# myshell-ai/OpenVoice

Measured on NVIDIA H100. Metric: audio_seconds_per_second, higher is better.
Workload: dtype f32 (3xFP16 split-precision tensor-core convs with fp32 accumulation, fp32 FFMA elsewhere)

## Files before the change

### include/ovc.h

```cpp
#ifndef OVC_B200_H
#define OVC_B200_H

#include <stddef.h>
#include <stdint.h>

#ifdef __cplusplus
extern "C" {
#endif

#define OVC_ABI_VERSION 17

#if defined(__GNUC__)
#define OVC_API __attribute__((visibility("default")))
#else
#define OVC_API
#endif

enum {
  OVC_OK = 0,
  OVC_ERR_INVALID = -1,
  OVC_ERR_CUDA = -2,
  OVC_ERR_STATE = -3,
  OVC_ERR_MISSING = -4,
  OVC_ERR_NOMEM = -5
};
// ... 154 lines not shown
                                      float* d_stats, int32_t* d_cum, float* d_g, int64_t* d_y_lengths, void* stream);
OVC_API int ovc_tts_decode_windows_tokens(ovc_ctx* ctx, const float* stats, const int32_t* cum, const float* g,
                                          const int64_t* y_lengths, int N, int T, const int64_t* row, const int64_t* frame0,
                                          const int64_t* len, int W, int Wmax, const uint64_t* seed, const int64_t* stream,
                                          const float* noise_scale, float* o, float* z_p, void* cuda_stream);

OVC_API int ovc_set_precision(ovc_ctx* ctx, int mode);

#define OVC_OPT_TTS_SIMPLE 2
#define OVC_OPT_GRAPH 3
#define OVC_OPT_PDL 5
#define OVC_OPT_BRANCHES 7
#define OVC_OPT_PAIR 8
#define OVC_OPT_PAIR_OCC 9
#define OVC_OPT_STAGED_EPI 10
OVC_API int ovc_set_option(ovc_ctx* ctx, int key, int value);

OVC_API int ovc_last_launch_count(const ovc_ctx* ctx);

OVC_API int ovc_graph_replays(const ovc_ctx* ctx);

OVC_API int ovc_profile_enable(ovc_ctx* ctx, int enable);
OVC_API int ovc_profile_read(ovc_ctx* ctx, double* ms, int64_t* launches, double* flops, double* bytes);
OVC_API int ovc_profile_detail(ovc_ctx* ctx, int max, char* names, double* ms, double* flops, double* bytes,
                               int* family);

OVC_API int ovc_debug_enable(ovc_ctx* ctx, int enable);
OVC_API int ovc_debug_fetch(ovc_ctx* ctx, const char* name, float* host_out, size_t max_floats,
                    int64_t* shape4 );

// ... 5 lines not shown
```

### openvoice_b200/_native.py

```python
from __future__ import annotations

import ctypes as C
import os
from typing import Dict, Iterable, Optional, Tuple

_HERE = os.path.dirname(os.path.abspath(__file__))
LIB_PATH = os.path.join(_HERE, "libovc_b200.so")

ABI_VERSION = 17
EXPORTS = (
    "ovc_abi_version", "ovc_last_error", "ovc_create", "ovc_destroy", "ovc_load_tensor",
    "ovc_finalize_weights", "ovc_workspace_floats", "ovc_voice_conversion", "ovc_last_launch_count",
    "ovc_profile_enable", "ovc_profile_read", "ovc_profile_detail", "ovc_debug_enable", "ovc_debug_fetch",
    "ovc_spectrogram", "ovc_convert_waveform", "ovc_set_precision", "ovc_reference_encoder",
    "ovc_tts_info", "ovc_tts_encode", "ovc_tts_decode", "ovc_set_option", "ovc_graph_replays",
    "ovc_reference_encoder_ragged", "ovc_resample", "ovc_resample_span", "ovc_voice_conversion_items",
    "ovc_convert_waveform_items", "ovc_tts_encode_items", "ovc_tts_decode_items", "ovc_philox_normals",
    "ovc_tts_encode_state", "ovc_tts_decode_windows", "ovc_spectrogram_ring", "ovc_splice",
    "ovc_tts_encode_state_rows", "ovc_tts_state_rows", "ovc_resample_plan", "ovc_resample_rings",
    "ovc_voice_conversion_frames", "ovc_convert_waveform_frames", "ovc_tone_track_expand",
    "ovc_tts_encode_g", "ovc_tts_encode_state_tokens", "ovc_tts_decode_windows_tokens", "ovc_tts_encode_state_rows_tokens",
    "ovc_tts_state_rows_tokens", "ovc_reference_encoder_stream", "ovc_reference_encoder_stream_state_floats",
    "ovc_generate_frames",
)
# ... 259 lines not shown
            _check(self.lib, rc, f"ovc_load_tensor({k})")
            (ignored if rc == 1 else used).append(k)
        self.finalized = False
        return used, ignored

    def finalize(self):
        _check(self.lib, self.lib.ovc_finalize_weights(self.handle), "ovc_finalize_weights")
        self.finalized = True

    def set_precision(self, mode: str):
        m = PRECISIONS[mode]
        _check(self.lib, self.lib.ovc_set_precision(self.handle, m), "ovc_set_precision")
        self.precision = mode

    def set_option(self, key: str, value: int):
        k = {"tts_simple": 2, "graph": 3, "pdl": 5, "branches": 7, "pair": 8, "pair_occ": 9, "staged_epi": 10}[key]
        _check(self.lib, self.lib.ovc_set_option(self.handle, k, int(value)), "ovc_set_option")

    def voice_conversion(self, spec, lengths, g_src, g_tgt, noise=None, tau: float = 0.3, seed: int = 0,
                         ragged: bool = False, latents: bool = True, stream=None, items: Optional[dict] = None, out=None):
        import torch
        assert spec.is_cuda and spec.dtype == torch.float32 and spec.is_contiguous()
        assert lengths.is_cuda and lengths.dtype == torch.int64 and lengths.is_contiguous()
        B, S, T = spec.shape
        gs, fs = se_arg(g_src, B, self.hp.gin_channels, T, "g_src")
        gt, ft = se_arg(g_tgt, B, self.hp.gin_channels, T, "g_tgt")
        if noise is not None:
            noise = noise.contiguous().float()
            assert tuple(noise.shape) == (B, self.hp.inter_channels, T)
        hop = self.hp.hop_length
        if out is not None:
# ... 486 lines not shown
```

### openvoice_b200/csrc/ovc_lib.cu

```cuda
#include <cuda_runtime.h>

#include <algorithm>
#include <cmath>
#include <cstdarg>
#include <cstdio>
#include <cstdlib>
#include <cstring>
#include <map>
#include <string>
#include <vector>

#include "../../include/ovc.h"
#include "ovc_convpack.h"
#include "ovc_small.cuh"
#include "ovc_tcconv.cuh"
#include "ovc_tts.cuh"
#include "ovc_refenc.cuh"
#include "ovc_resample.cuh"
#include "ovc_splice.h"
#include "ovc_variants.h"

namespace ovc {

static thread_local std::string g_err;
// ... 136 lines not shown
  ConvLayer dec_pre, dec_ups[4];
  ConvLayer rb_c1[12][3], rb_c2[12][3];
  TcLayer tc_c1[12][3], tc_c2[12][3], tc_ups[4], tc_pre;
  float* d_tcw = nullptr;
  std::vector<float> h_tcw;
  int precision = 0;
  bool tts_simple = false;
  bool use_graph = true;
  int use_pdl = 2;
  bool use_branches = true;
  int par_frames = 512;
  bool use_pair = true;
  bool use_pair_occ = true;
  bool use_staged_epi = true;
  bool pair_occ2_ok[TCN_N_OCC2] = {};
  cudaStream_t br_stream[2] = {nullptr, nullptr};
  cudaEvent_t br_ev[4] = {nullptr, nullptr, nullptr, nullptr};
  size_t post_w_off = 0;
  size_t cond_w_off = 0, cond_b_off = 0;
  int* d_cond_wrow = nullptr;
  int* d_cond_sel = nullptr;
  int cond_rows_out = 0;
  int cond_off_enc = 0, cond_off_fsrc = 0, cond_off_ftgt = 0, cond_off_dec = 0;
  int cond_off_enc_tc = 0, cond_off_fsrc_tc = 0, cond_off_ftgt_tc = 0;
  int* d_cond_cols[2][3] = {};
  int cond_pf_cols[2][3] = {};
  int cond_pf_off[2][3][4] = {};

  float2* d_tw = nullptr;
  float* d_win = nullptr;
// ... 426 lines not shown
  if (c->d_w) { cudaFree(c->d_w); c->d_w = nullptr; }
  c->w_floats = c->h_w.size();
  CK(cudaMalloc(&c->d_w, c->w_floats * sizeof(float)));
  CK(cudaMemcpy(c->d_w, c->h_w.data(), c->w_floats * sizeof(float), cudaMemcpyHostToDevice));
  if (c->d_tcw) { cudaFree(c->d_tcw); c->d_tcw = nullptr; }
  CK(cudaMalloc(&c->d_tcw, c->h_tcw.size() * sizeof(float)));
  CK(cudaMemcpy(c->d_tcw, c->h_tcw.data(), c->h_tcw.size() * sizeof(float), cudaMemcpyHostToDevice));
  c->h_tcw.clear();
  c->h_tcw.shrink_to_fit();
  for (int TN : {128, 64, 32})
    for (bool staged : {false, true}) {
      const TcKernel k = tc_conv_kernel(TN, staged), p = tc_pair_kernel(TN, TcPairOcc(), staged);
      CK(cudaFuncSetAttribute(k.fn, cudaFuncAttributeMaxDynamicSharedMemorySize, (int)k.smem));
      CK(cudaFuncSetAttribute(p.fn, cudaFuncAttributeMaxDynamicSharedMemorySize, (int)p.smem));
    }
  for (int i = 0; i < TCN_N_OCC2; ++i) {
    const TcKernel k = tc_pair_kernel(kTcPairOcc2[i].C, kTcPairOcc2[i].o);
    CK(cudaFuncSetAttribute(k.fn, cudaFuncAttributeMaxDynamicSharedMemorySize, (int)k.smem));
    int blocks = 0;
    CK(cudaOccupancyMaxActiveBlocksPerMultiprocessor(&blocks, k.fn, k.threads, k.smem));
    c->pair_occ2_ok[i] = blocks >= 2;
    if (blocks < 2)
      fprintf(stderr, "ovc: the C = %d conv-pair kernel with %d operand buffer(s) fits %d CTA(s) per SM, not 2; its pairs run "
              "one CTA per SM\n", kTcPairOcc2[i].C, kTcPairOcc2[i].o.nabuf, blocks);
  }
  if (c->d_cond_wrow) cudaFree(c->d_cond_wrow);
  if (c->d_cond_sel) cudaFree(c->d_cond_sel);
  CK(cudaMalloc(&c->d_cond_wrow, wrow.size() * sizeof(int)));
  CK(cudaMalloc(&c->d_cond_sel, sel.size() * sizeof(int)));
  CK(cudaMemcpy(c->d_cond_wrow, wrow.data(), wrow.size() * sizeof(int), cudaMemcpyHostToDevice));
// ... 169 lines not shown
  }
}

struct TcExtra {
  int epi = 0;
  const float* bias = nullptr;
  long long bias_bs = 0, bias_ts = 0;
  float* s = nullptr;
  int split = 0, first = 0;
  int y_ld = 0;
  bool use_lens_frames = false;
  const long long* lens_x = nullptr; bool has_lens_x = false;
  int grid_div = 1;
};
template <class... KArgs, class... Args>
static cudaError_t launch_ex(void (*kernel)(KArgs...), dim3 grid, int block, size_t smem, cudaStream_t st, bool pdl, Args&&... args) {
  cudaLaunchConfig_t cfg{};
  cfg.gridDim = grid;
  cfg.blockDim = dim3((unsigned)block, 1, 1);
  cfg.dynamicSmemBytes = smem;
  cfg.stream = st;
  cudaLaunchAttribute at[1];
  at[0].id = cudaLaunchAttributeProgrammaticStreamSerialization;
  at[0].val.programmaticStreamSerializationAllowed = 1;
  cfg.attrs = at;
  cfg.numAttrs = pdl ? 1 : 0;
  return cudaLaunchKernelEx(&cfg, kernel, std::forward<Args>(args)...);
}

static int launch_tc(Run& r, const TcLayer& T, const float* x, float* y, const float* res, int t_len, int mul, float slope,
                     float scale, int accumulate, int family, const TcExtra& ex = TcExtra()) {
  TcConvArgs a{};
  const int y_ld = ex.y_ld ? ex.y_ld : T.Ntot;
  a.x = x; a.x_bs = (long long)T.Cin * r.P * mul;
  a.w = reinterpret_cast<const uint16_t*>(r.c->d_tcw + T.w_off);
  a.bias = ex.bias ? ex.bias : r.c->d_tcw + T.b_off; a.bias_bs = ex.bias_bs; a.bias_ts = ex.bias_ts;
  a.y = y; a.y_bs = (long long)y_ld * r.P * mul; a.y_ld = y_ld;
  a.r = res;
  a.s = ex.s; a.s_bs = a.y_bs;
  a.epi = ex.epi; a.split = ex.split; a.first = ex.first;
  a.lens = ex.use_lens_frames ? r.lens : r.glens; a.tmax = r.Tmax; a.mul = mul;
  a.lens_x = ex.lens_x; a.has_lens_x = ex.has_lens_x ? 1 : 0;
  a.Cin = T.Cin; a.Ntot = T.Ntot; a.K = T.K; a.DIL = T.DIL;
  a.slope = slope; a.scale = scale; a.accumulate = accumulate;
  a.passes = r.c->precision == 2 ? 1 : 3;
  if (T.TN == 0) return fail(OVC_ERR_INVALID, "conv %d -> %d (k %d, dilation %d) does not fit the tensor-core kernels", T.Cin, T.Ntot, T.K, T.DIL);
  if (!(slope >= 0.f && slope <= 1.f)) return fail(OVC_ERR_INVALID, "leaky_relu slope %g outside [0, 1]", (double)slope);
  TRY(prof_begin(r));
  const TcGrid g = tc_grid(t_len, r.B, T.Ntot, T.TN, r.c->sm_count, ex.grid_div);
  const int n_tt = g.n_tt, total = g.total;
  dim3 pg((unsigned)g.grid_x, g.ncol, 1);
  const bool pdl = r.c->use_pdl == 1 || (r.c->use_pdl == 2 && ex.epi != 0);
  const TcKernel k = tc_conv_kernel(T.TN, r.c->use_staged_epi && tc_stage_pays(T.K, a.passes));
  CK(launch_ex(k.fn, pg, k.threads, k.smem, r.st, pdl, a, n_tt, total));
  CK(cudaGetLastError());
  r.c->launches++;
  const double units = (double)r.B * t_len;
  const int eff_k = family == 2 ? 2 : T.K;
  TRY(prof_end(r, T.TN == 128 ? V_TC128 : T.TN == 64 ? V_TC64 : V_TC32, family == 1 ? 1 : 0, 2.0 * T.Cin * T.Ntot * eff_k * units,
               4.0 * (T.Cin + T.Ntot * (1 + (res ? 1 : 0) + (accumulate ? 1 : 0))) * units, (T.Cin << 16) | (T.K << 8) | T.DIL));
  return OVC_OK;
}

static int launch_pair(Run& r, const TcLayer& T1, const TcLayer& T2, const float* x, float* y, int t_len, int mul, float slope,
                       float scale, int accumulate) {
  TcConvArgs a{};
  const int C = T1.TN;
  a.x = x; a.x_bs = (long long)C * r.P * mul;
  a.w = reinterpret_cast<const uint16_t*>(r.c->d_tcw + T1.w_off);
// ... 1 lines not shown
  a.bias = r.c->d_tcw + T1.b_off; a.bias2 = r.c->d_tcw + T2.b_off;
  a.y = y; a.y_bs = a.x_bs; a.y_ld = C;
  a.lens = r.glens; a.tmax = r.Tmax; a.mul = mul;
  a.Cin = C; a.Ntot = C; a.K = T1.K; a.DIL = T1.DIL;
  a.slope = slope; a.scale = scale; a.accumulate = accumulate;
  a.passes = r.c->precision == 2 ? 1 : 3;
  TcPairOcc o = r.c->use_pair_occ ? tc_pair_occ(T1, T2) : TcPairOcc();
  for (int i = 0; i < TCN_N_OCC2; ++i)
    if (o.occ == 2 && kTcPairOcc2[i].C == C && kTcPairOcc2[i].o.nabuf == o.nabuf && !r.c->pair_occ2_ok[i]) o = TcPairOcc();
  const TcKernel k = tc_pair_kernel(C, o, r.c->use_staged_epi && tc_stage_pays(T1.K, a.passes));
  if (!k.fn) return fail(OVC_ERR_INVALID, "no conv-pair kernel for C = %d at %d CTA(s) per SM, %d operand buffer(s)", C, o.occ, o.nabuf);
  const TcGrid g = tc_pair_grid(t_len, r.B, T1.K, r.c->sm_count, o.occ);
  const int n_tt = g.n_tt, total = g.total;
  TRY(prof_begin(r));
  dim3 pg((unsigned)g.grid_x, 1, 1);
  CK(launch_ex(k.fn, pg, k.threads, k.smem, r.st, false, a, n_tt, total));
  CK(cudaGetLastError());
  r.c->launches++;
  const double units = (double)r.B * t_len;
  TRY(prof_end(r, C == 128 ? V_TCPAIR128 : C == 64 ? V_TCPAIR64 : V_TCPAIR32, 1, 2.0 * 2.0 * C * C * T1.K * units, 4.0 * C * (2 + (accumulate ? 1 : 0)) * units,
               (C << 16) | (T1.K << 8) | T1.DIL));
  return OVC_OK;
}

static int launch_transpose(Run& r, const float* src, float* dst, int rows, int cols) {
  dim3 grid((cols + 31) / 32, (rows + 31) / 32, r.B);
  TRY(prof_begin(r));
  transpose_kernel<<<grid, 256, 0, r.st>>>(src, dst, rows, cols, (long long)rows * cols);
  CK(cudaGetLastError());
  r.c->launches++;
  TRY(prof_end(r, V_TRANSPOSE, 0, 0.0, 8.0 * rows * cols * r.B));
// ... 158 lines not shown
  }
  e->launches = c->launches;
  CK(cudaGraphLaunch(e->exec, st));
  c->graph_replays++;
  return OVC_OK;
}

static int set_call_params(ovc_ctx* c, uint64_t seed, float tau, const ItemParams& items, cudaStream_t st) {
  if (!c->d_callp) CK(cudaMalloc(&c->d_callp, sizeof(CallParams)));
  set_call_params_kernel<<<1, 1, 0, st>>>(c->d_callp, seed, tau, items);
  CK(cudaGetLastError());
  return OVC_OK;
}
static uintptr_t option_bits(const ovc_ctx* c) {
  return (uintptr_t)c->precision | ((uintptr_t)c->use_pdl << 15) | ((uintptr_t)c->use_branches << 14) | ((uintptr_t)c->use_pair << 17) |
         ((uintptr_t)c->use_pair_occ << 18) | ((uintptr_t)c->use_staged_epi << 19);
}

static int ensure_ws(ovc_ctx* c, const WsLayout& W, int B, int Tmax, cudaStream_t st) {
  if (W.total <= c->ws_floats) return OVC_OK;
  CK(cudaStreamSynchronize(st));
  drop_graphs(c);
  if (c->d_ws) CK(cudaFree(c->d_ws));
  c->d_ws = nullptr;
  c->ws_floats = 0;
  cudaError_t e = cudaMalloc(&c->d_ws, W.total * sizeof(float));
  if (e != cudaSuccess) {
    cudaGetLastError();
    return fail(OVC_ERR_NOMEM, "workspace of %.2f GB for B=%d Tmax=%d does not fit: %s", W.total * 4e-9, B, Tmax,
                cudaGetErrorString(e));
  }
// ... 1095 lines not shown
}

int ovc_set_option(ovc_ctx* c, int key, int value) {
  if (!c) return fail(OVC_ERR_INVALID, "null context");
  switch (key) {
    case OVC_OPT_TTS_SIMPLE: c->tts_simple = value != 0; return OVC_OK;
    case OVC_OPT_GRAPH: c->use_graph = value != 0; return OVC_OK;
    case OVC_OPT_PDL:
      if (value < 0 || value > 2) return fail(OVC_ERR_INVALID, "pdl must be 0, 1 or 2");
      c->use_pdl = value;
      return OVC_OK;
    case OVC_OPT_BRANCHES: c->use_branches = value != 0; return OVC_OK;
    case OVC_OPT_PAIR: c->use_pair = value != 0; return OVC_OK;
    case OVC_OPT_PAIR_OCC: c->use_pair_occ = value != 0; return OVC_OK;
    case OVC_OPT_STAGED_EPI: c->use_staged_epi = value != 0; return OVC_OK;
    default: return fail(OVC_ERR_INVALID, "unknown option %d", key);
  }
}

int ovc_last_launch_count(const ovc_ctx* c) { return c ? c->launches : 0; }

int ovc_graph_replays(const ovc_ctx* c) { return c ? c->graph_replays : 0; }

int ovc_profile_enable(ovc_ctx* c, int enable) {
  if (!c) return fail(OVC_ERR_INVALID, "null context");
  c->prof = enable != 0;
  c->ev_used = 0;
  c->ev_flops.clear();
  c->ev_bytes.clear();
  c->ev_variant.clear();
// ... 76 lines not shown
```

### openvoice_b200/csrc/ovc_tcconv.cuh

```cuda
#pragma once
#include "ovc_conv.cuh"
#include "ovc_tc.cuh"
#include "ovc_tcpack.h"

namespace ovc {

struct TcConvArgs {
  const float* x; long long x_bs;
  const uint16_t* w;
  const float* bias; long long bias_bs;
  float* y; long long y_bs; int y_ld;
  const float* r;
  float* s; long long s_bs;
  int epi;
  int split; int first;
  const long long* lens; int tmax; int mul;
  const long long* lens_x; int has_lens_x;
  int Cin; int Ntot; int K; int DIL;
  float slope; float scale; int accumulate;
  int passes;
  const uint16_t* w2; const float* bias2;
  long long bias_ts;
};

__device__ __forceinline__ void pdl_launch_dependents() { asm volatile("griddepcontrol.launch_dependents;" ::: "memory"); }
__device__ __forceinline__ void pdl_wait() { asm volatile("griddepcontrol.wait;" ::: "memory"); }

__device__ __forceinline__ void mbar_arrive(uint64_t* bar) {
  asm volatile("mbarrier.arrive.shared::cta.b64 _, [%0];" ::"r"(smem_u32(bar)) : "memory");
}
__device__ __forceinline__ void named_bar_sync(int id, int threads) {
  asm volatile("bar.sync %0, %1;" ::"r"(id), "r"(threads) : "memory");
}
__device__ __forceinline__ void named_bar_arrive(int id, int threads) {
  asm volatile("bar.arrive %0, %1;" ::"r"(id), "r"(threads) : "memory");
}

template <int TN>
__device__ __forceinline__ float tc_result(const float (&d)[TN], bool two, int j) {
  return two ? fmaf(d[TN / 2 + j], tc::kLoInv, d[j]) : d[j];
}

template <int TN, bool PF, class V>
__device__ __forceinline__ void tc_epilogue_body(const TcConvArgs& a, V v_at, int b, int t0, int n0, int lim, int row_a) {
  const int csub = (threadIdx.x & 3) * 2;
// ... 116 lines not shown
  static constexpr int SLOT_BYTES = 2 * 2 * TN * 16;
  static constexpr int A_BUF_BYTES = 2 * NKC * ROWS * 16;
  static constexpr int A2_BYTES = PAIR ? 2 * (TN / 8) * ROWS2 * 16 : 0;
  static constexpr int STAGE_BYTES = STAGED ? (TN / 2) * 256 * 4 : 0;
  static_assert(!STAGED || !PAIR || STAGE_BYTES <= A2_BYTES, "a pair's staging tile lies in its conv-2 operand");
  static constexpr int SBUF_BYTES = STAGED && !PAIR ? STAGE_BYTES : 0;
  static constexpr size_t SMEM_BYTES = 1024 + NABUF * A_BUF_BYTES + A2_BYTES + RING * SLOT_BYTES + SBUF_BYTES;
  static_assert(!PAIR || SMEM_BYTES == tc_pair_smem(TN, NABUF, RING), "tc_pair_smem");
  static_assert(SMEM_BYTES <= (OCC == 1 ? 232448 : TCN_SMEM_OCC2), "shared memory budget");
  static_assert((2 * NABUF + 2 * RING + 2) * 8 <= 1024, "barrier area");
  static constexpr int PROD_REGS = OCC == 1 && !STAGED ? 56 : 32, MMA_REGS = STAGED ? 184 : OCC == 1 ? 224 : 104;
  static constexpr int STORE_REGS = 112;
  static_assert(128 * PROD_REGS + 256 * MMA_REGS + (STAGED ? 128 * STORE_REGS : 0) <= 65536 / OCC, "register budget");
};

template <int TN, bool PAIR, int OCC = 1, int NAB = 2, bool STAGED = false>
__global__ void __launch_bounds__(TcnCfg<TN, PAIR, OCC, NAB, STAGED>::THREADS, OCC) tcconv_kernel(const TcConvArgs a, int n_tt, int total) {
  using Cfg = TcnCfg<TN, PAIR, OCC, NAB, STAGED>;
  constexpr int ROWS = Cfg::ROWS, ROWS2 = Cfg::ROWS2, NABUF = Cfg::NABUF, RING = Cfg::RING, NKC = Cfg::NKC;
  extern __shared__ __align__(128) unsigned char smem_raw[];
  uint64_t* bars = reinterpret_cast<uint64_t*>(smem_raw);
  uint64_t *a_full = bars, *a_empty = bars + NABUF, *b_full = a_empty + NABUF, *b_empty = b_full + RING;
  uint64_t *s_full = b_empty + RING, *s_empty = s_full + 1;
  unsigned char* abuf = smem_raw + 1024;
  unsigned char* a2buf = abuf + NABUF * Cfg::A_BUF_BYTES;
  unsigned char* bring = a2buf + Cfg::A2_BYTES;
  float* stage = reinterpret_cast<float*>(PAIR ? a2buf : bring + RING * Cfg::SLOT_BYTES);

  const int tid = threadIdx.x, lane = tid & 31;
  const int warp = __shfl_sync(0xffffffffu, tid >> 5, 0);
  const int H1 = (a.K - 1) / 2 * a.DIL;
  const int H2 = PAIR ? (a.K - 1) / 2 : 0;
  const int R = 128 - 2 * H2;
  const int rows8 = (128 + 2 * H1 + 7) & ~7;
  const int nq = a.Cin / Cfg::KCH;
  const int n_slots = (a.Cin / 16) * a.K;
  const int n_w = PAIR ? 2 * n_slots : n_slots;
  const bool resident = n_w <= RING;
  if (H1 > TCN_HMAX || (PAIR && 128 + 2 * H2 > ROWS2)) __trap();
  constexpr uint32_t BYTES = Cfg::SLOT_BYTES;

  if (tid == 0) {
    for (int i = 0; i < NABUF; ++i) { mbar_init(&a_full[i], TCN_NCT); mbar_init(&a_empty[i], 2); }
    for (int i = 0; i < RING; ++i) { mbar_init(&b_full[i], 1); mbar_init(&b_empty[i], 2); }
    if (STAGED) { mbar_init(s_full, 256); mbar_init(s_empty, 128); }
    fence_mbar_init();
  }
  if (PAIR) {
    for (int i = tid; i < Cfg::A2_BYTES / 16; i += Cfg::THREADS) reinterpret_cast<uint4*>(a2buf)[i] = make_uint4(0u, 0u, 0u, 0u);
    asm volatile("fence.proxy.async.shared::cta;" ::: "memory");
  }
  __syncthreads();
  pdl_launch_dependents();
  if (warp != 0) pdl_wait();

#define TCN_FOR_TILES                                                                                   \
  for (int tile = blockIdx.x; tile < total; tile += gridDim.x) {                                        \
    const int b = tile / n_tt, t0 = (tile % n_tt) * R;                                                  \
    const int lim = (a.lens ? (int)min((long long)a.tmax, a.lens[b]) : a.tmax) * a.mul;                 \
    const int lim_x = a.has_lens_x ? (int)min((long long)a.tmax, a.lens_x[b]) * a.mul : lim;            \
    (void)lim_x;                                                                                        \
    if (t0 >= lim) continue;

  if (warp < 4) {
    tc::regs_dealloc<Cfg::PROD_REGS>();
    if (warp == 0) {
      if (lane == 0) {
        const unsigned char* wt = reinterpret_cast<const unsigned char*>(a.w) + (size_t)blockIdx.y * n_slots * BYTES;
        if (resident) {
          for (int it = 0; it < n_w; ++it) {
            const unsigned char* src = it < n_slots ? wt + (size_t)it * BYTES
                                                    : reinterpret_cast<const unsigned char*>(a.w2) + (size_t)(it - n_slots) * BYTES;
            mbar_expect_tx(&b_full[it], BYTES);
            tma_bulk_g2s(bring + it * BYTES, src, BYTES, &b_full[it]);
          }
          for (int it = 0; it < n_w; ++it) mbar_wait(&b_full[it], 0u);
        } else {
          int slot = 0;
          uint32_t phase = 1;
          TCN_FOR_TILES
            (void)b;
            for (int it = 0; it < n_w; ++it) {
              const unsigned char* src = it < n_slots ? wt + (size_t)it * BYTES
                                                      : reinterpret_cast<const unsigned char*>(a.w2) + (size_t)(it - n_slots) * BYTES;
              mbar_wait(&b_empty[slot], phase);
              mbar_expect_tx(&b_full[slot], BYTES);
              tma_bulk_g2s(bring + slot * BYTES, src, BYTES, &b_full[slot]);
              if (++slot == RING) { slot = 0; phase ^= 1; }
            }
          }
        }
      }
    } else {
      const int pt = tid - 32;
      const int items = rows8 * NKC;
      int buf = 0;
      uint32_t ephase = 1;
      TCN_FOR_TILES
        const float* xb = a.x + (size_t)b * a.x_bs;
        const int r0 = t0 - H2 - H1;
        for (int q = 0; q < nq; ++q) {
          mbar_wait(&a_empty[buf], ephase);
          unsigned char* ah = abuf + buf * Cfg::A_BUF_BYTES;
          unsigned char* al = ah + NKC * ROWS * 16;
          constexpr int PB = 2;
          for (int i0 = pt; i0 < items; i0 += TCN_NCT * PB) {
            float4 v0[PB], v1[PB];
#pragma unroll
            for (int u = 0; u < PB; ++u) {
              const int i = i0 + TCN_NCT * u;
              const int row = i >> 2, kc = i & 3;
              const int t = r0 + row;
              v0[u] = make_float4(0.f, 0.f, 0.f, 0.f);
              v1[u] = v0[u];
              if (i < items && t >= 0 && t < lim_x) {
                const float4* src = reinterpret_cast<const float4*>(xb + (size_t)t * a.Cin + q * Cfg::KCH + kc * 8);
                v0[u] = src[0];
                v1[u] = src[1];
              }
            }
#pragma unroll
            for (int u = 0; u < PB; ++u) {
              const int i = i0 + TCN_NCT * u;
              if (i >= items) break;
              const int row = i >> 2, kc = i & 3;
              uint4 hi, lo;
              tc::split_f16x8(v0[u], v1[u], a.slope, hi, lo);
              *reinterpret_cast<uint4*>(ah + (kc * ROWS + row) * 16) = hi;
              *reinterpret_cast<uint4*>(al + (kc * ROWS + row) * 16) = lo;
            }
          }
          asm volatile("fence.proxy.async.shared::cta;" ::: "memory");
          mbar_arrive(&a_full[buf]);
          if (++buf == NABUF) { buf = 0; ephase ^= 1; }
        }
      }
    }
  } else if (STAGED && warp >= 12) {
    tc::regs_dealloc<Cfg::STORE_REGS>();
    const int st = tid & 127;
    uint32_t phase = 0;
    TCN_FOR_TILES
      if (PAIR) named_bar_arrive(1, 384);
      mbar_wait(s_full, phase);
      phase ^= 1;
#pragma unroll 1
      for (int h = 0; h < 2; ++h) {
        const float* sv = stage + h * 128 + st;
        const auto v_at = [&](int j) { return sv[j * 256]; };
        const int row_a = 64 * h + 16 * (warp & 3) + (lane >> 2);
        if constexpr (PAIR) tc_epilogue_v<TN>(tc_pair_epilogue_args(a, TN), v_at, b, t0, 0, min(lim, t0 + R), row_a);
        else tc_epilogue_v<TN>(a, v_at, b, t0, blockIdx.y * TN, lim, row_a);
      }
      if (!PAIR) mbar_arrive(s_empty);
    }
  } else {
    tc::regs_alloc<Cfg::MMA_REGS>();
    const int wg = (warp >> 2) - 1;
    const bool leader = (tid & 127) == 0;
    const int row_a = 64 * wg + 16 * (warp & 3) + (lane >> 2);
    constexpr uint32_t LBO_A = ROWS * 16, LBO_A2 = ROWS2 * 16, LBO_B = 2 * TN * 16, SBO = 128;
    constexpr uint32_t A_LO16 = (NKC * ROWS * 16) >> 4, A2_LO16 = ((TN / 8) * ROWS2 * 16) >> 4, SLOT16 = BYTES >> 4;
    const uint64_t a_proto = tc::make_desc(0, LBO_A, SBO), b_proto = tc::make_desc(0, LBO_B, SBO);
    const uint64_t b_ring = b_proto + (tc::smem_addr(bring) >> 4);
    const bool three = a.passes == 3;
    float d[TN];
#pragma unroll
    for (int i = 0; i < TN; ++i) d[i] = 0.f;
    const auto stage_tile = [&]() {
#pragma unroll
      for (int j = 0; j < TN / 2; ++j) stage[j * 256 + tid - 128] = tc_result<TN>(d, three, j);
      mbar_arrive(s_full);
    };
    uint32_t sphase = 1;
    (void)sphase;
    if (resident)
      for (int it = 0; it < n_w; ++it) mbar_wait(&b_full[it], 0u);
    int slot = 0, buf = 0;
    uint32_t bphase = 0, aphase = 0;
    TCN_FOR_TILES
      (void)lim_x;
      bool first = true;
      if (resident) slot = 0;
      for (int q = 0; q < nq; ++q) {
        mbar_wait(&a_full[buf], aphase);
        tc::fence_regs(d);
        tc::wgmma_fence();
        int prev = -1;
        for (int j = 0; j < 2; ++j) {
          uint64_t a_cur = a_proto + ((tc::smem_addr(abuf + buf * Cfg::A_BUF_BYTES) + 64 * wg * 16 + 2 * j * LBO_A) >> 4);
          for (int tap = 0; tap < a.K; ++tap) {
            if (!resident) mbar_wait(&b_full[slot], bphase);
            tc_mma_step<TN>(d, a_cur, a_cur + A_LO16, b_ring + (uint32_t)slot * SLOT16, three, first);
            tc::wgmma_commit();
            if (!resident) {
              tc::wgmma_wait<1>();
              if (leader && prev >= 0) mbar_arrive(&b_empty[prev]);
              prev = slot;
            }
            first = false;
            a_cur += a.DIL;
            if (++slot == RING) { slot = 0; bphase ^= 1; }
          }
        }
        tc::wgmma_wait<0>();
        tc::fence_regs(d);
        if (leader) {
          if (prev >= 0) mbar_arrive(&b_empty[prev]);
          mbar_arrive(&a_empty[buf]);
        }
        if (++buf == NABUF) { buf = 0; aphase ^= 1; }
      }
      if constexpr (!PAIR) {
        if constexpr (STAGED) {
          mbar_wait(s_empty, sphase);
          sphase ^= 1;
          stage_tile();
        } else {
          tc_epilogue<TN>(a, d, b, t0, blockIdx.y * TN, lim, row_a);
        }
      } else {
        named_bar_sync(1, STAGED ? 384 : 256);
        unsigned char* a2h = a2buf;
        unsigned char* a2l = a2buf + (TN / 8) * ROWS2 * 16;
// ... 46 lines not shown
          }
        }
        tc::wgmma_commit();
        tc::wgmma_wait<0>();
        tc::fence_regs(d);
        if (leader && prev >= 0) mbar_arrive(&b_empty[prev]);
        if constexpr (STAGED) {
          named_bar_sync(3, 256);
          stage_tile();
        } else {
          tc_epilogue<TN>(tc_pair_epilogue_args(a, TN), d, b, t0, 0, min(lim, t0 + R), row_a);
        }
      }
    }
  }
#undef TCN_FOR_TILES
}

struct TcKernel {
  void (*fn)(TcConvArgs, int, int) = nullptr;
  size_t smem = 0;
  int threads = 0;
};
using TcPairKernel = TcKernel;
template <int TN, bool PAIR, int OCC = 1, int NAB = 2, bool STAGED = false>
inline TcKernel tc_kernel() {
  using Cfg = TcnCfg<TN, PAIR, OCC, NAB, STAGED>;
  return {tcconv_kernel<TN, PAIR, OCC, NAB, STAGED>, Cfg::SMEM_BYTES, Cfg::THREADS};
}
inline bool tc_stage_pays(int K, int passes) { return passes * K >= 15; }
inline TcKernel tc_conv_kernel(int TN, bool staged) {
  if (TN == 128) return staged ? tc_kernel<128, false, 1, 2, true>() : tc_kernel<128, false>();
  if (TN == 64) return tc_kernel<64, false>();
  if (TN == 32) return tc_kernel<32, false>();
  return {};
}
inline TcKernel tc_pair_kernel(int C, TcPairOcc o, bool staged = false) {
  if (o.occ == 1 && o.nabuf == 2) {
    if (C == 128) return staged ? tc_kernel<128, true, 1, 2, true>() : tc_kernel<128, true>();
    if (C == 64) return tc_kernel<64, true>();
    if (C == 32) return tc_kernel<32, true>();
  } else if (o.occ == 2) {
    if (C == 32 && o.nabuf == 2) return tc_kernel<32, true, 2, 2>();
    if (C == 32 && o.nabuf == 1) return tc_kernel<32, true, 2, 1>();
    if (C == 64 && o.nabuf == 1) return tc_kernel<64, true, 2, 1>();
  }
  return {};
}
constexpr int TCN_N_OCC2 = 3;
constexpr struct { int C; TcPairOcc o; } kTcPairOcc2[TCN_N_OCC2] = {{32, {2, 2}}, {32, {2, 1}}, {64, {2, 1}}};

// ... 57 lines not shown
```

### openvoice_b200/csrc/ovc_tcpack.h

```cpp
#pragma once
#include <cuda_fp16.h>
#include <stddef.h>
#include <stdint.h>

#include <algorithm>

namespace ovc {

constexpr int TCN_HMAX = 25;
constexpr int TCN_ROWS2 = 146;

constexpr int tc_ring_slots(int TN, bool pair) {
  return pair ? (TN == 32 ? 44 : TN == 64 ? 24 : 12) : (TN == 32 ? 22 : 12);
}

struct TcGeom {
  int Cin = 0, Ntot = 0, K = 0, DIL = 1, TN = 0;
};

inline int tc_tile_n(int Ntot, int Cin, int K, int DIL) {
  if (Ntot <= 0 || Cin <= 0 || K <= 0 || DIL <= 0) return 0;
  if (Ntot % 32 || Cin % 32 || (K - 1) / 2 * DIL > TCN_HMAX) return 0;
  return Ntot % 128 == 0 ? 128 : (Ntot % 64 == 0 ? 64 : 32);
}
// ... 44 lines not shown
  if (!(T1.TN == 32 || T1.TN == 64)) return false;
  const int ring = tc_ring_slots(T1.TN, true);
  return T1.Ntot == T1.TN && T1.Cin == T1.TN && T2.Ntot == T1.TN && T2.Cin == T1.TN && T2.TN == T1.TN && T2.K == T1.K &&
         T2.DIL == 1 && (T1.K - 1) / 2 * T1.DIL <= TCN_HMAX && 2 * (T1.Cin / 16) * T1.K <= ring && T1.K <= 5;
}

inline bool tc_pair_fuses(const TcGeom& T1, const TcGeom& T2) {
  if (!(T1.TN == 32 || T1.TN == 64 || T1.TN == 128)) return false;
  return T1.Ntot == T1.TN && T1.Cin == T1.TN && T2.Ntot == T1.TN && T2.Cin == T1.TN && T2.TN == T1.TN && T2.K == T1.K &&
         T2.DIL == 1 && (T1.K - 1) / 2 * T1.DIL <= TCN_HMAX && 128 + 2 * ((T2.K - 1) / 2) <= TCN_ROWS2;
}

struct TcGrid {
  int n_tt = 0, total = 0, grid_x = 0, ncol = 0;
};
inline TcGrid tc_grid(int t_len, int B, int Ntot, int TN, int sm_count, int grid_div) {
  TcGrid g;
  g.n_tt = (t_len + 127) / 128;
  g.total = g.n_tt * B;
  g.ncol = Ntot / TN;
  const int per_col = std::max(1, sm_count / g.ncol / std::max(1, grid_div));
  g.grid_x = std::min(g.total, per_col);
  return g;
}
inline TcGrid tc_pair_grid(int t_len, int B, int K, int sm_count, int occ = 1) {
  TcGrid g;
  const int R = 128 - (K - 1);
  g.n_tt = (t_len + R - 1) / R;
  g.total = g.n_tt * B;
  g.ncol = 1;
  g.grid_x = std::min(g.total, occ * sm_count);
  return g;
}

constexpr size_t tc_pair_smem(int TN, int nabuf, int ring) {
  return 1024 + (size_t)nabuf * 2 * 4 * 194 * 16 + (size_t)2 * (TN / 8) * TCN_ROWS2 * 16 + (size_t)ring * 2 * 2 * TN * 16;
}
constexpr size_t TCN_SMEM_OCC2 = (233472 - 2 * 1024) / 2;
// ... 19 lines not shown
```

Before: 2426.

## Share activation tiles across output-column CTAs via thread-block cluster DSMEM multicast

Groups the CTAs that handle different output-channel columns of the same time tile into a thread-block cluster (2-4 wide). Each CTA's producer warps convert only a slice of the input rows to split fp16, then push that slice to peer CTAs' shared memory with bulk shared::cluster copies. Cross-CTA mbarriers coordinate buffer reuse. This is meant to cut redundant global loads and hi/lo conversion work when several column CTAs read the same activations. In exchange it adds cluster synchronisation, remote-barrier latency and co-scheduling constraints. It is enabled by default for selected kernel shapes (3-pass with K=5, or K=1).

```diff
diff --git a/include/ovc.h b/include/ovc.h
--- a/include/ovc.h
+++ b/include/ovc.h
@@ -8,7 +8,7 @@
 extern "C" {
 #endif
 
-#define OVC_ABI_VERSION 17
+#define OVC_ABI_VERSION 18
 
 #if defined(__GNUC__)
 #define OVC_API __attribute__((visibility("default")))
@@ -193,6 +193,7 @@
 #define OVC_OPT_PAIR 8
 #define OVC_OPT_PAIR_OCC 9
 #define OVC_OPT_STAGED_EPI 10
+#define OVC_OPT_CLUSTER_FEED 11
 OVC_API int ovc_set_option(ovc_ctx* ctx, int key, int value);
 
 OVC_API int ovc_last_launch_count(const ovc_ctx* ctx);
diff --git a/openvoice_b200/_native.py b/openvoice_b200/_native.py
--- a/openvoice_b200/_native.py
+++ b/openvoice_b200/_native.py
@@ -7,7 +7,7 @@
 _HERE = os.path.dirname(os.path.abspath(__file__))
 LIB_PATH = os.path.join(_HERE, "libovc_b200.so")
 
-ABI_VERSION = 17
+ABI_VERSION = 18
 EXPORTS = (
     "ovc_abi_version", "ovc_last_error", "ovc_create", "ovc_destroy", "ovc_load_tensor",
     "ovc_finalize_weights", "ovc_workspace_floats", "ovc_voice_conversion", "ovc_last_launch_count",
@@ -297,7 +297,7 @@
         self.precision = mode
 
     def set_option(self, key: str, value: int):
-        k = {"tts_simple": 2, "graph": 3, "pdl": 5, "branches": 7, "pair": 8, "pair_occ": 9, "staged_epi": 10}[key]
+        k = {"tts_simple": 2, "graph": 3, "pdl": 5, "branches": 7, "pair": 8, "pair_occ": 9, "staged_epi": 10, "cluster_feed": 11}[key]
         _check(self.lib, self.lib.ovc_set_option(self.handle, k, int(value)), "ovc_set_option")
 
     def voice_conversion(self, spec, lengths, g_src, g_tgt, noise=None, tau: float = 0.3, seed: int = 0,
diff --git a/openvoice_b200/csrc/ovc_lib.cu b/openvoice_b200/csrc/ovc_lib.cu
--- a/openvoice_b200/csrc/ovc_lib.cu
+++ b/openvoice_b200/csrc/ovc_lib.cu
@@ -174,6 +174,8 @@
   bool use_pair_occ = true;
   bool use_staged_epi = true;
   bool pair_occ2_ok[TCN_N_OCC2] = {};
+  bool use_cluster_feed = true;
+  int tc_max_clusters[4][5] = {};
   cudaStream_t br_stream[2] = {nullptr, nullptr};
   cudaEvent_t br_ev[4] = {nullptr, nullptr, nullptr, nullptr};
   size_t post_w_off = 0;
@@ -630,6 +632,26 @@
       CK(cudaFuncSetAttribute(k.fn, cudaFuncAttributeMaxDynamicSharedMemorySize, (int)k.smem));
       CK(cudaFuncSetAttribute(p.fn, cudaFuncAttributeMaxDynamicSharedMemorySize, (int)p.smem));
     }
+  for (int kind = 0; kind < 4; ++kind)
+    for (int cl = 2; cl <= 4; ++cl) {
+      const TcKernel k = tc_conv_kernel(kTcClusterTN[kind], kind == 1, cl);
+      CK(cudaFuncSetAttribute(k.fn, cudaFuncAttributeMaxDynamicSharedMemorySize, (int)k.smem));
+      cudaLaunchConfig_t cfg{};
+      cfg.gridDim = dim3(1, (unsigned)cl, 1);
+      cfg.blockDim = dim3((unsigned)k.threads, 1, 1);
+      cfg.dynamicSmemBytes = k.smem;
+      cudaLaunchAttribute at[1];
+      at[0].id = cudaLaunchAttributeClusterDimension;
+      at[0].val.clusterDim.x = 1; at[0].val.clusterDim.y = (unsigned)cl; at[0].val.clusterDim.z = 1;
+      cfg.attrs = at;
+      cfg.numAttrs = 1;
+      int n = 0;
+      if (cudaOccupancyMaxActiveClusters(&n, k.fn, &cfg) != cudaSuccess) {
+        cudaGetLastError();
+        n = 0;
+      }
+      c->tc_max_clusters[kind][cl] = n;
+    }
   for (int i = 0; i < TCN_N_OCC2; ++i) {
     const TcKernel k = tc_pair_kernel(kTcPairOcc2[i].C, kTcPairOcc2[i].o);
     CK(cudaFuncSetAttribute(k.fn, cudaFuncAttributeMaxDynamicSharedMemorySize, (int)k.smem));
@@ -829,17 +851,26 @@
   int grid_div = 1;
 };
 template <class... KArgs, class... Args>
-static cudaError_t launch_ex(void (*kernel)(KArgs...), dim3 grid, int block, size_t smem, cudaStream_t st, bool pdl, Args&&... args) {
+static cudaError_t launch_ex(void (*kernel)(KArgs...), dim3 grid, int block, size_t smem, cudaStream_t st, bool pdl, int cluster_y,
+                             Args&&... args) {
   cudaLaunchConfig_t cfg{};
   cfg.gridDim = grid;
   cfg.blockDim = dim3((unsigned)block, 1, 1);
   cfg.dynamicSmemBytes = smem;
   cfg.stream = st;
-  cudaLaunchAttribute at[1];
-  at[0].id = cudaLaunchAttributeProgrammaticStreamSerialization;
-  at[0].val.programmaticStreamSerializationAllowed = 1;
+  cudaLaunchAttribute at[2];
+  int n = 0;
+  if (pdl) {
+    at[n].id = cudaLaunchAttributeProgrammaticStreamSerialization;
+    at[n++].val.programmaticStreamSerializationAllowed = 1;
+  }
+  if (cluster_y > 1) {
+    at[n].id = cudaLaunchAttributeClusterDimension;
+    at[n].val.clusterDim.x = 1; at[n].val.clusterDim.y = (unsigned)cluster_y; at[n].val.clusterDim.z = 1;
+    ++n;
+  }
   cfg.attrs = at;
-  cfg.numAttrs = pdl ? 1 : 0;
+  cfg.numAttrs = n;
   return cudaLaunchKernelEx(&cfg, kernel, std::forward<Args>(args)...);
 }
 
@@ -862,12 +893,16 @@
   if (T.TN == 0) return fail(OVC_ERR_INVALID, "conv %d -> %d (k %d, dilation %d) does not fit the tensor-core kernels", T.Cin, T.Ntot, T.K, T.DIL);
   if (!(slope >= 0.f && slope <= 1.f)) return fail(OVC_ERR_INVALID, "leaky_relu slope %g outside [0, 1]", (double)slope);
   TRY(prof_begin(r));
-  const TcGrid g = tc_grid(t_len, r.B, T.Ntot, T.TN, r.c->sm_count, ex.grid_div);
+  const bool staged = r.c->use_staged_epi && tc_stage_pays(T.K, a.passes);
+  const int (&max_clusters)[5] = r.c->tc_max_clusters[tc_cluster_kind(T.TN, staged)];
+  const int cl = tc_cluster_use(T.Ntot / T.TN, ex.grid_div, r.c->use_cluster_feed && tc_cluster_pays(T.Cin, T.K, T.TN, a.passes),
+                                max_clusters);
+  const TcGrid g = tc_grid(t_len, r.B, T.Ntot, T.TN, r.c->sm_count, ex.grid_div, cl, max_clusters[cl]);
   const int n_tt = g.n_tt, total = g.total;
   dim3 pg((unsigned)g.grid_x, g.ncol, 1);
   const bool pdl = r.c->use_pdl == 1 || (r.c->use_pdl == 2 && ex.epi != 0);
-  const TcKernel k = tc_conv_kernel(T.TN, r.c->use_staged_epi && tc_stage_pays(T.K, a.passes));
-  CK(launch_ex(k.fn, pg, k.threads, k.smem, r.st, pdl, a, n_tt, total));
+  const TcKernel k = tc_conv_kernel(T.TN, staged, cl);
+  CK(launch_ex(k.fn, pg, k.threads, k.smem, r.st, pdl, cl, a, n_tt, total));
   CK(cudaGetLastError());
   r.c->launches++;
   const double units = (double)r.B * t_len;
@@ -899,7 +934,7 @@
   const int n_tt = g.n_tt, total = g.total;
   TRY(prof_begin(r));
   dim3 pg((unsigned)g.grid_x, 1, 1);
-  CK(launch_ex(k.fn, pg, k.threads, k.smem, r.st, false, a, n_tt, total));
+  CK(launch_ex(k.fn, pg, k.threads, k.smem, r.st, false, 1, a, n_tt, total));
   CK(cudaGetLastError());
   r.c->launches++;
   const double units = (double)r.B * t_len;
@@ -1088,7 +1123,7 @@
 }
 static uintptr_t option_bits(const ovc_ctx* c) {
   return (uintptr_t)c->precision | ((uintptr_t)c->use_pdl << 15) | ((uintptr_t)c->use_branches << 14) | ((uintptr_t)c->use_pair << 17) |
-         ((uintptr_t)c->use_pair_occ << 18) | ((uintptr_t)c->use_staged_epi << 19);
+         ((uintptr_t)c->use_pair_occ << 18) | ((uintptr_t)c->use_staged_epi << 19) | ((uintptr_t)c->use_cluster_feed << 20);
 }
 
 static int ensure_ws(ovc_ctx* c, const WsLayout& W, int B, int Tmax, cudaStream_t st) {
@@ -2214,6 +2249,7 @@
     case OVC_OPT_PAIR: c->use_pair = value != 0; return OVC_OK;
     case OVC_OPT_PAIR_OCC: c->use_pair_occ = value != 0; return OVC_OK;
     case OVC_OPT_STAGED_EPI: c->use_staged_epi = value != 0; return OVC_OK;
+    case OVC_OPT_CLUSTER_FEED: c->use_cluster_feed = value != 0; return OVC_OK;
     default: return fail(OVC_ERR_INVALID, "unknown option %d", key);
   }
 }
diff --git a/openvoice_b200/csrc/ovc_tcconv.cuh b/openvoice_b200/csrc/ovc_tcconv.cuh
--- a/openvoice_b200/csrc/ovc_tcconv.cuh
+++ b/openvoice_b200/csrc/ovc_tcconv.cuh
@@ -29,6 +29,46 @@
 __device__ __forceinline__ void mbar_arrive(uint64_t* bar) {
   asm volatile("mbarrier.arrive.shared::cta.b64 _, [%0];" ::"r"(smem_u32(bar)) : "memory");
 }
+__device__ __forceinline__ uint32_t cluster_ctarank() {
+  uint32_t r;
+  asm volatile("mov.u32 %0, %%cluster_ctarank;" : "=r"(r));
+  return r;
+}
+__device__ __forceinline__ uint32_t mapa_shared(uint32_t addr, uint32_t rank) {
+  uint32_t r;
+  asm volatile("mapa.shared::cluster.u32 %0, %1, %2;" : "=r"(r) : "r"(addr), "r"(rank));
+  return r;
+}
+__device__ __forceinline__ void cluster_sync_all() {
+  asm volatile("barrier.cluster.arrive.release;\n\tbarrier.cluster.wait.acquire;" ::: "memory");
+}
+__device__ __forceinline__ void mbar_arrive_remote(uint32_t cluster_addr) {
+  asm volatile("mbarrier.arrive.shared::cluster.b64 _, [%0];" ::"r"(cluster_addr) : "memory");
+}
+__device__ __forceinline__ void mbar_wait_cluster(uint64_t* bar, uint32_t parity) {
+  const auto try_wait = [&]() {
+    uint32_t ok;
+    asm volatile(
+        "{\n\t.reg .pred p;\n\t"
+        "mbarrier.try_wait.parity.acquire.cluster.shared::cta.b64 p, [%1], %2;\n\t"
+        "selp.u32 %0, 1, 0, p;\n\t}"
+        : "=r"(ok)
+        : "r"(smem_u32(bar)), "r"(parity)
+        : "memory");
+    return ok != 0;
+  };
+  if (try_wait()) return;
+  const long long t0 = clock64();
+  while (!try_wait()) {
+    if (clock64() - t0 > 4000000000LL) __trap();
+  }
+}
+__device__ __forceinline__ void bulk_s2s_cluster(uint32_t dst, const void* src, uint32_t bytes, uint32_t bar) {
+  asm volatile("cp.async.bulk.shared::cluster.shared::cta.mbarrier::complete_tx::bytes [%0], [%1], %2, [%3];" ::"r"(dst),
+               "r"(smem_u32(src)), "r"(bytes), "r"(bar)
+               : "memory");
+}
+
 __device__ __forceinline__ void named_bar_sync(int id, int threads) {
   asm volatile("bar.sync %0, %1;" ::"r"(id), "r"(threads) : "memory");
 }
@@ -175,9 +215,10 @@
   static_assert(128 * PROD_REGS + 256 * MMA_REGS + (STAGED ? 128 * STORE_REGS : 0) <= 65536 / OCC, "register budget");
 };
 
-template <int TN, bool PAIR, int OCC = 1, int NAB = 2, bool STAGED = false>
+template <int TN, bool PAIR, int OCC = 1, int NAB = 2, bool STAGED = false, int CL = 1>
 __global__ void __launch_bounds__(TcnCfg<TN, PAIR, OCC, NAB, STAGED>::THREADS, OCC) tcconv_kernel(const TcConvArgs a, int n_tt, int total) {
   using Cfg = TcnCfg<TN, PAIR, OCC, NAB, STAGED>;
+  static_assert(CL == 1 || (!PAIR && OCC == 1), "clusters: single convs at one CTA per SM");
   constexpr int ROWS = Cfg::ROWS, ROWS2 = Cfg::ROWS2, NABUF = Cfg::NABUF, RING = Cfg::RING, NKC = Cfg::NKC;
   extern __shared__ __align__(128) unsigned char smem_raw[];
   uint64_t* bars = reinterpret_cast<uint64_t*>(smem_raw);
@@ -199,10 +240,13 @@
   const int n_w = PAIR ? 2 * n_slots : n_slots;
   const bool resident = n_w <= RING;
   if (H1 > TCN_HMAX || (PAIR && 128 + 2 * H2 > ROWS2)) __trap();
+  if (CL > 1 && gridDim.y % CL) __trap();
   constexpr uint32_t BYTES = Cfg::SLOT_BYTES;
+  constexpr int PROD_REGS = CL > 1 && STAGED ? 48 : Cfg::PROD_REGS, STORE_REGS = CL > 1 && STAGED ? 96 : Cfg::STORE_REGS;
+  static_assert(128 * PROD_REGS + 256 * Cfg::MMA_REGS + (STAGED ? 128 * STORE_REGS : 0) <= 65536 / OCC, "register budget");
 
   if (tid == 0) {
-    for (int i = 0; i < NABUF; ++i) { mbar_init(&a_full[i], TCN_NCT); mbar_init(&a_empty[i], 2); }
+    for (int i = 0; i < NABUF; ++i) { mbar_init(&a_full[i], TCN_NCT); mbar_init(&a_empty[i], 2 * CL); }
     for (int i = 0; i < RING; ++i) { mbar_init(&b_full[i], 1); mbar_init(&b_empty[i], 2); }
     if (STAGED) { mbar_init(s_full, 256); mbar_init(s_empty, 128); }
     fence_mbar_init();
@@ -211,7 +255,8 @@
     for (int i = tid; i < Cfg::A2_BYTES / 16; i += Cfg::THREADS) reinterpret_cast<uint4*>(a2buf)[i] = make_uint4(0u, 0u, 0u, 0u);
     asm volatile("fence.proxy.async.shared::cta;" ::: "memory");
   }
-  __syncthreads();
+  if constexpr (CL > 1) cluster_sync_all();
+  else __syncthreads();
   pdl_launch_dependents();
   if (warp != 0) pdl_wait();
 
@@ -224,7 +269,7 @@
     if (t0 >= lim) continue;
 
   if (warp < 4) {
-    tc::regs_dealloc<Cfg::PROD_REGS>();
+    tc::regs_dealloc<PROD_REGS>();
     if (warp == 0) {
       if (lane == 0) {
         const unsigned char* wt = reinterpret_cast<const unsigned char*>(a.w) + (size_t)blockIdx.y * n_slots * BYTES;
@@ -254,14 +299,19 @@
       }
     } else {
       const int pt = tid - 32;
-      const int items = rows8 * NKC;
+      const int crank = CL > 1 ? (int)cluster_ctarank() : 0;
+      const int s0 = CL > 1 ? tc_cluster_share(rows8, CL, crank) : 0;
+      const int s1 = CL > 1 ? tc_cluster_share(rows8, CL, crank + 1) : rows8;
+      const int items = (s1 - s0) * NKC;
+      const uint32_t peer_bytes = (uint32_t)(rows8 - (s1 - s0)) * 16u * 2u * NKC;
       int buf = 0;
       uint32_t ephase = 1;
       TCN_FOR_TILES
         const float* xb = a.x + (size_t)b * a.x_bs;
         const int r0 = t0 - H2 - H1;
         for (int q = 0; q < nq; ++q) {
-          mbar_wait(&a_empty[buf], ephase);
+          if constexpr (CL > 1) mbar_wait_cluster(&a_empty[buf], ephase);
+          else mbar_wait(&a_empty[buf], ephase);
           unsigned char* ah = abuf + buf * Cfg::A_BUF_BYTES;
           unsigned char* al = ah + NKC * ROWS * 16;
           constexpr int PB = 2;
@@ -270,7 +320,7 @@
 #pragma unroll
             for (int u = 0; u < PB; ++u) {
               const int i = i0 + TCN_NCT * u;
-              const int row = i >> 2, kc = i & 3;
+              const int row = s0 + (i >> 2), kc = i & 3;
               const int t = r0 + row;
               v0[u] = make_float4(0.f, 0.f, 0.f, 0.f);
               v1[u] = v0[u];
@@ -284,7 +334,7 @@
             for (int u = 0; u < PB; ++u) {
               const int i = i0 + TCN_NCT * u;
               if (i >= items) break;
-              const int row = i >> 2, kc = i & 3;
+              const int row = s0 + (i >> 2), kc = i & 3;
               uint4 hi, lo;
               tc::split_f16x8(v0[u], v1[u], a.slope, hi, lo);
               *reinterpret_cast<uint4*>(ah + (kc * ROWS + row) * 16) = hi;
@@ -292,13 +342,33 @@
             }
           }
           asm volatile("fence.proxy.async.shared::cta;" ::: "memory");
-          mbar_arrive(&a_full[buf]);
+          if constexpr (CL > 1) {
+            named_bar_sync(4, TCN_NCT);
+            if (pt == 0) {
+              mbar_expect_tx(&a_full[buf], peer_bytes);
+              const uint32_t bytes = (uint32_t)items * 4u;
+#pragma unroll 1
+              for (int p = 1; p < CL; ++p) {
+                const uint32_t peer = (uint32_t)((crank + p) % CL);
+                const uint32_t bar = mapa_shared(smem_u32(&a_full[buf]), peer);
+#pragma unroll 1
+                for (int j = 0; j < 2 * NKC; ++j) {
+                  const unsigned char* src = ah + (j * ROWS + s0) * 16;
+                  bulk_s2s_cluster(mapa_shared(smem_u32(src), peer), src, bytes, bar);
+                }
+              }
+            } else {
+              mbar_arrive(&a_full[buf]);
+            }
+          } else {
+            mbar_arrive(&a_full[buf]);
+          }
           if (++buf == NABUF) { buf = 0; ephase ^= 1; }
         }
       }
     }
   } else if (STAGED && warp >= 12) {
-    tc::regs_dealloc<Cfg::STORE_REGS>();
+    tc::regs_dealloc<STORE_REGS>();
     const int st = tid & 127;
     uint32_t phase = 0;
     TCN_FOR_TILES
@@ -323,7 +393,8 @@
     constexpr uint32_t LBO_A = ROWS * 16, LBO_A2 = ROWS2 * 16, LBO_B = 2 * TN * 16, SBO = 128;
     constexpr uint32_t A_LO16 = (NKC * ROWS * 16) >> 4, A2_LO16 = ((TN / 8) * ROWS2 * 16) >> 4, SLOT16 = BYTES >> 4;
     const uint64_t a_proto = tc::make_desc(0, LBO_A, SBO), b_proto = tc::make_desc(0, LBO_B, SBO);
-    const uint64_t b_ring = b_proto + (tc::smem_addr(bring) >> 4);
+    const auto desc_addr = [](const void* p) { return CL > 1 ? tc::smem_addr(p) & 0x3FFFFu : tc::smem_addr(p); };
+    const uint64_t b_ring = b_proto + (desc_addr(bring) >> 4);
     const bool three = a.passes == 3;
     float d[TN];
 #pragma unroll
@@ -349,7 +420,7 @@
         tc::wgmma_fence();
         int prev = -1;
         for (int j = 0; j < 2; ++j) {
-          uint64_t a_cur = a_proto + ((tc::smem_addr(abuf + buf * Cfg::A_BUF_BYTES) + 64 * wg * 16 + 2 * j * LBO_A) >> 4);
+          uint64_t a_cur = a_proto + ((desc_addr(abuf + buf * Cfg::A_BUF_BYTES) + 64 * wg * 16 + 2 * j * LBO_A) >> 4);
           for (int tap = 0; tap < a.K; ++tap) {
             if (!resident) mbar_wait(&b_full[slot], bphase);
             tc_mma_step<TN>(d, a_cur, a_cur + A_LO16, b_ring + (uint32_t)slot * SLOT16, three, first);
@@ -368,7 +439,11 @@
         tc::fence_regs(d);
         if (leader) {
           if (prev >= 0) mbar_arrive(&b_empty[prev]);
-          mbar_arrive(&a_empty[buf]);
+          if constexpr (CL > 1) {
+            for (int p = 0; p < CL; ++p) mbar_arrive_remote(mapa_shared(smem_u32(&a_empty[buf]), (uint32_t)p));
+          } else {
+            mbar_arrive(&a_empty[buf]);
+          }
         }
         if (++buf == NABUF) { buf = 0; aphase ^= 1; }
       }
@@ -445,6 +520,7 @@
       }
     }
   }
+  if constexpr (CL > 1) cluster_sync_all();
 #undef TCN_FOR_TILES
 }
 
@@ -454,18 +530,30 @@
   int threads = 0;
 };
 using TcPairKernel = TcKernel;
-template <int TN, bool PAIR, int OCC = 1, int NAB = 2, bool STAGED = false>
+template <int TN, bool PAIR, int OCC = 1, int NAB = 2, bool STAGED = false, int CL = 1>
 inline TcKernel tc_kernel() {
   using Cfg = TcnCfg<TN, PAIR, OCC, NAB, STAGED>;
-  return {tcconv_kernel<TN, PAIR, OCC, NAB, STAGED>, Cfg::SMEM_BYTES, Cfg::THREADS};
+  return {tcconv_kernel<TN, PAIR, OCC, NAB, STAGED, CL>, Cfg::SMEM_BYTES, Cfg::THREADS};
 }
 inline bool tc_stage_pays(int K, int passes) { return passes * K >= 15; }
-inline TcKernel tc_conv_kernel(int TN, bool staged) {
-  if (TN == 128) return staged ? tc_kernel<128, false, 1, 2, true>() : tc_kernel<128, false>();
-  if (TN == 64) return tc_kernel<64, false>();
-  if (TN == 32) return tc_kernel<32, false>();
+template <int CL>
+inline TcKernel tc_conv_kernel_cl(int TN, bool staged) {
+  if (TN == 128) return staged ? tc_kernel<128, false, 1, 2, true, CL>() : tc_kernel<128, false, 1, 2, false, CL>();
+  if (TN == 64) return tc_kernel<64, false, 1, 2, false, CL>();
+  if (TN == 32) return tc_kernel<32, false, 1, 2, false, CL>();
   return {};
 }
+inline TcKernel tc_conv_kernel(int TN, bool staged, int cl = 1) {
+  switch (cl) {
+    case 1: return tc_conv_kernel_cl<1>(TN, staged);
+    case 2: return tc_conv_kernel_cl<2>(TN, staged);
+    case 3: return tc_conv_kernel_cl<3>(TN, staged);
+    case 4: return tc_conv_kernel_cl<4>(TN, staged);
+    default: return {};
+  }
+}
+constexpr int kTcClusterTN[4] = {128, 128, 64, 32};
+inline int tc_cluster_kind(int TN, bool staged) { return TN == 128 ? (staged ? 1 : 0) : TN == 64 ? 2 : 3; }
 inline TcKernel tc_pair_kernel(int C, TcPairOcc o, bool staged = false) {
   if (o.occ == 1 && o.nabuf == 2) {
     if (C == 128) return staged ? tc_kernel<128, true, 1, 2, true>() : tc_kernel<128, true>();
diff --git a/openvoice_b200/csrc/ovc_tcpack.h b/openvoice_b200/csrc/ovc_tcpack.h
--- a/openvoice_b200/csrc/ovc_tcpack.h
+++ b/openvoice_b200/csrc/ovc_tcpack.h
@@ -82,14 +82,30 @@
 struct TcGrid {
   int n_tt = 0, total = 0, grid_x = 0, ncol = 0;
 };
-inline TcGrid tc_grid(int t_len, int B, int Ntot, int TN, int sm_count, int grid_div) {
+inline TcGrid tc_grid(int t_len, int B, int Ntot, int TN, int sm_count, int grid_div, int cl = 1, int max_clusters = 0) {
   TcGrid g;
   g.n_tt = (t_len + 127) / 128;
   g.total = g.n_tt * B;
   g.ncol = Ntot / TN;
-  const int per_col = std::max(1, sm_count / g.ncol / std::max(1, grid_div));
+  const int per_col = cl > 1 ? std::max(1, max_clusters * cl / g.ncol) : std::max(1, sm_count / g.ncol / std::max(1, grid_div));
   g.grid_x = std::min(g.total, per_col);
   return g;
+}
+
+constexpr int tc_cluster_share(int rows8, int cl, int r) { return rows8 * r / cl; }
+inline bool tc_cluster_pays(int Cin, int K, int TN, int passes) {
+  (void)Cin; (void)TN;
+  return passes == 3 ? K == 5 : K == 1;
+}
+inline int tc_cluster_cols(int ncol, int grid_div, bool on) {
+  if (!on || grid_div != 1 || ncol < 2) return 1;
+  for (int cl : {4, 3, 2})
+    if (ncol % cl == 0) return cl;
+  return 1;
+}
+inline int tc_cluster_use(int ncol, int grid_div, bool on, const int (&max_clusters)[5]) {
+  const int cl = tc_cluster_cols(ncol, grid_div, on);
+  return cl > 1 && max_clusters[cl] > 0 ? cl : 1;
 }
 inline TcGrid tc_pair_grid(int t_len, int B, int K, int sm_count, int occ = 1) {
   TcGrid g;
```

Result: no change. 2440 (median of 6 runs) (+0.5%).
